# PierfrancescoArdino/C2M

Hardware: AMD Instinct MI355X
Metric: generator train-step frames/sec at 128x256x7 (higher is better)
Workload: dtype f32; 1 GPU; BASELINE configs[1]: 128x256, 7-frame clips (2 in + 5 predicted), batch 8/GPU, fp32, generator fwd+bwd only (no D), VGG loss on, random-init weights; global_batch=8, parallelism=single

## Files before the change

c2m_amd/csrc/conv_common.h:

```cpp
#pragma once
#include "common.h"
#include "dtype.h"
#include "conv_store.h"
#include "conv_types.h"

struct ConvP {
    const float* A;
    const float* X;
    float* Y;
    const float* bias;
    const int4* ktab;
    int M, nk, lda;
    int Npix, To, Ho, Wo;
    int Ti, Hi, Wi;
    int st, sh, sw;
    int in_sc;
    long in_sn, in_st, in_sh;
    long out_sn, out_sc, out_st, out_sh, out_sw, out_off;
    long slab_stride;
    unsigned x_bytes;
    float* Y2;
    int ps_t, ps_y, ps_x, po_t, po_y, po_x, lo_t, lo_y, lo_x, ext_t, ext_y, ext_x;
    long y2_sn, y2_sc, y2_st, y2_sh;
    int iy0, ix0, pty[3], ptx[3], nchunks, cin;
    int ksteps_per_split;
    int reflect, is3d;
    int act;
    float slope;
    int ncls, splits, ktab_cls;
    int xh, yh;
    long a_cls;
    long out_off_c[8];
    int po_c[8][3];
    int g8_nch, g8_ntaps, g8_CB, g8_Mpad;
    unsigned g8_a_bytes, g8_plane_bytes;
    int g8_dbg;
};

struct WgradP {
    const float* dY;
    const float* X;
    float* slab;
    const int4* jtab;
    int M, J;
    int Npix, To, Ho, Wo, Ti, Hi, Wi, st, sh, sw;
    int in_sc;
    long in_sn, in_st, in_sh;
    long dy_sn, dy_sc;
    int pix_per_split;
    int reflect, is3d;
    unsigned x_bytes, dy_bytes;
};

__device__ __forceinline__ int spatial_off(const int4 tp, int ots, int oys, int oxs, int Ti, int Hi, int Wi, int in_st,
                                           int in_sh, int reflect, int is3d) {
    int it = is3d ? ots + tp.x : 0, iy = oys + tp.y, ix = oxs + tp.z;
    bool ok = tp.w != 0;
    if (reflect) {
        if (is3d) { it = it < 0 ? -it : it; it = it >= Ti ? 2 * Ti - 2 - it : it; }
        iy = iy < 0 ? -iy : iy; iy = iy >= Hi ? 2 * Hi - 2 - iy : iy;
        ix = ix < 0 ? -ix : ix; ix = ix >= Wi ? 2 * Wi - 2 - ix : ix;
    } else {
        ok = ok && (unsigned)iy < (unsigned)Hi && (unsigned)ix < (unsigned)Wi;
        if (is3d) ok = ok && (unsigned)it < (unsigned)Ti;
    }
    return ok ? it * in_st + iy * in_sh + ix : -1;
}

template <class P>
__device__ __forceinline__ void decompose_pix(int pix, const P& p, int& n, int& ot, int& oy, int& ox) {
    ox = pix % p.Wo; int r = pix / p.Wo;
    oy = r % p.Ho;   r = r / p.Ho;
    ot = r % p.To;   n = r / p.To;
}

int c2m_launch_gather_nc8(const ConvP& p, int variant, int splits, hipStream_t s);
int c2m_launch_patch(const ConvP& p, int splits, hipStream_t s);
int c2m_launch_patch_bf16(const ConvP& p, int splits, hipStream_t s);
int c2m_launch_thin_fwd(const ConvP& p, int ns, hipStream_t s);
int c2m_launch_thin_rows(const ConvP& p, int kw, int ns, int ntg, int Cin, int xdesc, hipStream_t s);
int c2m_launch_thin_wgrad_rows(const WgradP& p, int kw, int NS, int ntg, int Cin, int ngroups, int S, hipStream_t s);
int c2m_launch_thin_wgrad(WgradP p, int NS, int ngroups, int S, hipStream_t s);
```

c2m_amd/csrc/conv_igemm.hip:

```cpp
#include "conv_common.h"

template <int BM, int BN, int WGM, int WGN, int NS, int U, bool BF = false>
__global__ __launch_bounds__(256) void conv_igemm_kernel(const ConvP p) {
    constexpr int BK = 16, CK = BK / NS, BKU = BK * U;
    constexpr int TM = BM / WGM, TN = BN / WGN, MI = TM / 32, NI = TN / 32;
    constexpr int LDA_S = BM + 4, LDB_S = BN;
    constexpr int BROWS = 256 / BN;
    constexpr int BPASS = BK / BROWS;
    constexpr int A_F4 = BM * BK / 4;
    constexpr int APASS = (A_F4 + 255) / 256;
    static_assert(WGM * WGN == 4 && BN >= 64 && CK % BROWS == 0, "tile");
    static_assert(!BF || BROWS <= 2, "bf16 slot packing is written for BN = 128 / 256");
    __shared__ float sA[BF ? 1 : 2][BF ? 1 : BKU][BF ? 1 : LDA_S];
    __shared__ float sB[BF ? 1 : 2][BF ? 1 : BKU][BF ? 1 : LDB_S];
    __shared__ uint4 hA[BF ? 2 * U * 2 * BM : 1];
    __shared__ uint4 hB[BF ? 2 * U * 2 * BN : 1];

    const int tid = threadIdx.x, lane = tid & 63, wave = tid >> 6;
    const int wm = wave / WGN, wn = wave % WGN;
    const C2mBlock blk = c2m_xcd_block((unsigned)(p.Npix + BN - 1) / BN, (unsigned)(p.M + BM - 1) / BM, 1);
    const int m0 = blk.y * BM, n0 = blk.x * BN;
    const int cls = p.ncls > 1 ? (int)blk.z / p.splits : 0;
    const int split = p.ncls > 1 ? (int)blk.z - cls * p.splits : (int)blk.z;
    const float* __restrict__ Acls = p.A + cls * p.a_cls;
    const int4* __restrict__ ktab = p.ktab + cls * p.ktab_cls;
    const int kt_beg = split * p.ksteps_per_split;
    int kt_end = kt_beg + p.ksteps_per_split; kt_end = kt_end < p.nk ? kt_end : p.nk;

    const int bp = tid % BN;
    const int brow0 = __builtin_amdgcn_readfirstlane(tid / BN);
    int pn, pt, py, px;
    {
        int pix = n0 + bp; pix = pix < p.Npix ? pix : p.Npix - 1;
        decompose_pix(pix, p, pn, pt, py, px);
    }
    const int ots = pt * p.st, oys = py * p.sh, oxs = px * p.sw;
    const int in_st = (int)p.in_st, in_sh = (int)p.in_sh;

    const int akq = (tid & 3) * 4;
    const int arow = tid >> 2;

    f32x16 acc[MI][NI];
#pragma unroll
    for (int i = 0; i < MI; ++i)
#pragma unroll
        for (int j = 0; j < NI; ++j)
#pragma unroll
            for (int r = 0; r < 16; ++r) acc[i][j][r] = 0.f;

    float4 ra[U][APASS];
    float rb[BF ? 1 : U][BF ? 1 : BPASS];
    unsigned short rh[BF ? U : 1][BF ? BPASS : 1];
    constexpr int XES = BF ? 2 : 4;

    const float* __restrict__ aptr[APASS];
#pragma unroll
    for (int s = 0; s < APASS; ++s) {
        int row = m0 + arow + s * 64; row = row < p.M ? row : p.M - 1;
        aptr[s] = Acls + (long)row * p.lda + akq;
    }
    int4 t_hdr, t_tap[NS];
    auto fetch_table = [&](int kt) {
        const int4* __restrict__ kd = ktab + (long)kt * (1 + NS);
        t_hdr = kd[0];
#pragma unroll
        for (int q = 0; q < NS; ++q) t_tap[q] = kd[1 + q];
    };

    const __amdgpu_buffer_rsrc_t xrsrc = __builtin_amdgcn_make_buffer_rsrc(const_cast<float*>(p.X), 0, p.x_bytes, 0x00020000);
    const unsigned img_byte = (unsigned)(pn * (int)p.in_sn) * (unsigned)XES;
    auto load_step = [&](int kt, float4 (&fa)[APASS], float (&fb)[BF ? 1 : BPASS], unsigned short (&fh)[BF ? BPASS : 1]) {
        const bool real = kt < kt_end;
#pragma unroll
        for (int s = 0; s < APASS; ++s) {
            if (A_F4 >= 256 || arow + s * 64 < BM)
                fa[s] = real ? *reinterpret_cast<const float4*>(aptr[s] + kt * BK) : make_float4(0.f, 0.f, 0.f, 0.f);
        }
        const int4 hdr = t_hdr;
        unsigned vo[NS];
#pragma unroll
        for (int q = 0; q < NS; ++q) {
            const int so = spatial_off(t_tap[q], ots, oys, oxs, p.Ti, p.Hi, p.Wi, in_st, in_sh, p.reflect, p.is3d);
            vo[q] = (real && so >= 0) ? img_byte + (unsigned)so * (unsigned)XES : C2M_OOB;
        }
#pragma unroll
        for (int s = 0; s < BPASS; ++s) {
            const int slot = (s * BROWS) / CK;
            const int cc = (s * BROWS) % CK + brow0;
            const int soff = (hdr.x + cc * p.in_sc) * XES;
            if constexpr (BF) fh[s] = __builtin_amdgcn_raw_buffer_load_b16(xrsrc, vo[slot], soff, 0);
            else fb[s] = __builtin_bit_cast(float, __builtin_amdgcn_raw_buffer_load_b32(xrsrc, vo[slot], soff, 0));
        }
        fetch_table(kt + 1 < p.nk ? kt + 1 : p.nk - 1);
    };
    auto load_tile = [&](int kt) {
#pragma unroll
        for (int u = 0; u < U; ++u) load_step(kt + u, ra[u], rb[BF ? 0 : u], rh[BF ? u : 0]);
    };
    auto store_tile = [&](int buf) {
#pragma unroll
        for (int u = 0; u < U; ++u) {
            if constexpr (BF) {
                __bf16* __restrict__ a8 = reinterpret_cast<__bf16*>(hA) + (long)((buf * U + u) * 2) * BM * 8;
#pragma unroll
                for (int s = 0; s < APASS; ++s) {
                    const int r = arow + s * 64;
                    if (A_F4 >= 256 || r < BM) {
                        const float4 v = ra[u][s];
                        if constexpr (BROWS == 1) {
                            bf16x4 q = {(__bf16)v.x, (__bf16)v.y, (__bf16)v.z, (__bf16)v.w};
                            *reinterpret_cast<bf16x4*>(a8 + ((akq >> 3) * BM + r) * 8 + (akq & 7)) = q;
                        } else {
                            bf16x2 e = {(__bf16)v.x, (__bf16)v.z}, o = {(__bf16)v.y, (__bf16)v.w};
                            *reinterpret_cast<bf16x2*>(a8 + (0 * BM + r) * 8 + (akq >> 1)) = e;
                            *reinterpret_cast<bf16x2*>(a8 + (1 * BM + r) * 8 + (akq >> 1)) = o;
                        }
                    }
                }
                uint4* __restrict__ b8 = hB + (long)((buf * U + u) * 2) * BN;
#pragma unroll
                for (int hh = 0; hh < BPASS / 8; ++hh) {
                    bf16x8 q;
#pragma unroll
                    for (int e = 0; e < 8; ++e) q[e] = __builtin_bit_cast(__bf16, rh[u][hh * 8 + e]);
                    const int h = BROWS == 1 ? hh : brow0;
                    b8[h * BN + bp] = __builtin_bit_cast(uint4, q);
                }
            } else {
#pragma unroll
                for (int s = 0; s < APASS; ++s) {
                    int r = arow + s * 64;
                    if (A_F4 >= 256 || r < BM) {
                        sA[buf][u * BK + akq + 0][r] = ra[u][s].x; sA[buf][u * BK + akq + 1][r] = ra[u][s].y;
                        sA[buf][u * BK + akq + 2][r] = ra[u][s].z; sA[buf][u * BK + akq + 3][r] = ra[u][s].w;
                    }
                }
#pragma unroll
                for (int s = 0; s < BPASS; ++s) sB[buf][u * BK + brow0 + s * BROWS][bp] = rb[u][s];
            }
        }
    };

    if (kt_beg < kt_end) {
        fetch_table(kt_beg);
        load_tile(kt_beg);
        store_tile(0);
    }
    __syncthreads();
    int cur = 0;
    for (int kt = kt_beg; kt < kt_end; kt += U) {
        const bool more = kt + U < kt_end;
        constexpr bool IL = !BF && U == 1 && BM < 128;
        if (!IL && more) load_tile(kt + U);
        if constexpr (BF) {
#pragma unroll
            for (int u = 0; u < U; ++u) {
                const uint4* __restrict__ a8 = hA + (long)((cur * U + u) * 2 + (lane >> 5)) * BM;
                const uint4* __restrict__ b8 = hB + (long)((cur * U + u) * 2 + (lane >> 5)) * BN;
                bf16x8 a[MI], b[NI];
#pragma unroll
                for (int i = 0; i < MI; ++i) a[i] = __builtin_bit_cast(bf16x8, a8[wm * TM + i * 32 + (lane & 31)]);
#pragma unroll
                for (int j = 0; j < NI; ++j) b[j] = __builtin_bit_cast(bf16x8, b8[wn * TN + j * 32 + (lane & 31)]);
#pragma unroll
                for (int i = 0; i < MI; ++i)
#pragma unroll
                    for (int j = 0; j < NI; ++j)
                        acc[i][j] = __builtin_amdgcn_mfma_f32_32x32x16_bf16(a[i], b[j], acc[i][j], 0, 0, 0);
            }
        } else if constexpr (IL) {
            float a[BK / 2][MI], b[BK / 2][NI];
#pragma unroll
            for (int kk = 0; kk < BK / 2; ++kk) {
                const int krow = kk * 2 + (lane >> 5);
#pragma unroll
                for (int i = 0; i < MI; ++i) a[kk][i] = sA[cur][krow][wm * TM + i * 32 + (lane & 31)];
#pragma unroll
                for (int j = 0; j < NI; ++j) b[kk][j] = sB[cur][krow][wn * TN + j * 32 + (lane & 31)];
            }
            {
                const int ktl = more ? kt + 1 : kt;
#pragma unroll
                for (int s2 = 0; s2 < APASS; ++s2)
                    if (A_F4 >= 256 || arow + s2 * 64 < BM) ra[0][s2] = *reinterpret_cast<const float4*>(aptr[s2] + ktl * BK);
                const int4 hdr = t_hdr;
                unsigned vo[NS];
#pragma unroll
                for (int q = 0; q < NS; ++q) {
                    const int so = spatial_off(t_tap[q], ots, oys, oxs, p.Ti, p.Hi, p.Wi, in_st, in_sh, p.reflect, p.is3d);
                    vo[q] = so >= 0 ? img_byte + (unsigned)so * 4u : C2M_OOB;
                }
#pragma unroll
                for (int s2 = 0; s2 < BPASS; ++s2) {
                    const int slot = (s2 * BROWS) / CK;
                    const int cc = (s2 * BROWS) % CK + brow0;
                    rb[0][s2] = __builtin_bit_cast(float, __builtin_amdgcn_raw_buffer_load_b32(
                        xrsrc, vo[slot], (hdr.x + cc * p.in_sc) * 4, 0));
                }
            }
#pragma unroll
            for (int kk = 0; kk < BK / 2; ++kk)
#pragma unroll
                for (int i = 0; i < MI; ++i)
#pragma unroll
                    for (int j = 0; j < NI; ++j)
                        acc[i][j] = __builtin_amdgcn_mfma_f32_32x32x2f32(a[kk][i], b[kk][j], acc[i][j], 0, 0, 0);
            constexpr int NMF = (BK / 2) * MI * NI, RPM = (MI + NI + MI * NI - 1) / (MI * NI);
            __builtin_amdgcn_sched_group_barrier(0x100, 2 * (MI + NI), 0);
#pragma unroll
            for (int g = 0; g < NMF; ++g) {
                __builtin_amdgcn_sched_group_barrier(0x008, 1, 0);
                __builtin_amdgcn_sched_group_barrier(0x100, RPM, 0);
                __builtin_amdgcn_sched_group_barrier(0x020, 1, 0);
                __builtin_amdgcn_sched_group_barrier(0x002, 3, 0);
                __builtin_amdgcn_sched_group_barrier(0x004, 2, 0);
            }
            __builtin_amdgcn_sched_barrier(0);
            fetch_table(kt + 2 < p.nk ? kt + 2 : p.nk - 1);
        } else
#pragma unroll
        for (int u = 0; u < U; ++u) {
            float a[BK / 2][MI], b[BK / 2][NI];
#pragma unroll
            for (int kk = 0; kk < BK / 2; ++kk) {
                const int krow = u * BK + kk * 2 + (lane >> 5);
#pragma unroll
                for (int i = 0; i < MI; ++i) a[kk][i] = sA[cur][krow][wm * TM + i * 32 + (lane & 31)];
#pragma unroll
                for (int j = 0; j < NI; ++j) b[kk][j] = sB[cur][krow][wn * TN + j * 32 + (lane & 31)];
            }
#ifdef C2M_IGEMM_SERIAL_FRAGS
            __builtin_amdgcn_sched_barrier(0);
#endif
#pragma unroll
            for (int kk = 0; kk < BK / 2; ++kk) {
#pragma unroll
                for (int i = 0; i < MI; ++i)
#pragma unroll
                    for (int j = 0; j < NI; ++j)
                        acc[i][j] = __builtin_amdgcn_mfma_f32_32x32x2f32(a[kk][i], b[kk][j], acc[i][j], 0, 0, 0);
            }
#ifndef C2M_IGEMM_SERIAL_FRAGS
            {
                constexpr int NMF = (BK / 2) * MI * NI, RPM = (MI + NI + MI * NI - 1) / (MI * NI);
                __builtin_amdgcn_sched_group_barrier(0x100, MI + NI, 0);
#pragma unroll
                for (int g = 0; g < NMF; ++g) {
                    __builtin_amdgcn_sched_group_barrier(0x008, 1, 0);
                    __builtin_amdgcn_sched_group_barrier(0x100, RPM, 0);
                }
            }
#endif
            __builtin_amdgcn_sched_barrier(0);
        }
        if (more) store_tile(cur ^ 1);
        __syncthreads();
        cur ^= 1;
    }

    const bool direct = p.splits == 1;
    const bool yh = BF && p.yh && direct;
    const int yes = yh ? 2 : 4;
    float* __restrict__ Yb = yh ? reinterpret_cast<float*>(reinterpret_cast<bf16_t*>(p.Y) + p.out_off_c[cls])
                                : p.Y + (long)split * p.slab_stride + p.out_off_c[cls];
    const int po_t = p.po_c[cls][0], po_y = p.po_c[cls][1], po_x = p.po_c[cls][2];
    {
        const int row0 = __builtin_amdgcn_readfirstlane(m0 + wm * TM);
        if (row0 + MI * 32 <= p.M) {
            unsigned voff[NI], voff2[NI];
            bool ring = false;
#pragma unroll
            for (int j = 0; j < NI; ++j) {
                const int pix = n0 + wn * TN + j * 32 + (lane & 31);
                int n, ot, oy, ox;
                decompose_pix(pix < p.Npix ? pix : 0, p, n, ot, oy, ox);
                const long e = (long)n * p.out_sn + (long)ot * p.out_st + (long)oy * p.out_sh + (long)ox * p.out_sw +
                               4L * (lane >> 5) * p.out_sc;
                voff[j] = pix < p.Npix ? (unsigned)(e * yes) : 0x80000000u;
                voff2[j] = 0x80000000u;
                if (p.Y2) {
                    const int tp = ot * p.ps_t + po_t - p.lo_t, yp = oy * p.ps_y + po_y - p.lo_y,
                              xp = ox * p.ps_x + po_x - p.lo_x;
                    if (pix < p.Npix && (unsigned)tp < (unsigned)p.ext_t && (unsigned)yp < (unsigned)p.ext_y &&
                        (unsigned)xp < (unsigned)p.ext_x) {
                        const long e2 = (long)n * p.y2_sn + (long)tp * p.y2_st + (long)yp * p.y2_sh + xp +
                                        4L * (lane >> 5) * p.y2_sc;
                        voff2[j] = (unsigned)(e2 * yes);
                        voff[j] = 0x80000000u;
                    }
                }
                ring = ring || voff[j] != 0x80000000u;
            }
            if (p.Y2) c2m_store_tile_fast<MI, NI>(acc, p.Y2, voff2, row0, p.y2_sc, nullptr, false, 0, 0.f, lane, yh);
            if (!p.Y2 || __any(ring))
                c2m_store_tile_fast<MI, NI>(acc, Yb, voff, row0, p.out_sc, p.bias, direct, p.act, p.slope, lane, yh);
            return;
        }
    }
#pragma unroll
    for (int j = 0; j < NI; ++j) {
        const int pix = n0 + wn * TN + j * 32 + (lane & 31);
        if (pix >= p.Npix) continue;
        int n, ot, oy, ox;
        decompose_pix(pix, p, n, ot, oy, ox);
        float* ybase = Yb;
        long yidx = (long)n * p.out_sn + (long)ot * p.out_st + (long)oy * p.out_sh + (long)ox * p.out_sw;
        long row_stride = p.out_sc;
        if (p.Y2) {
            const int tp = ot * p.ps_t + po_t - p.lo_t, yp = oy * p.ps_y + po_y - p.lo_y,
                      xp = ox * p.ps_x + po_x - p.lo_x;
            if ((unsigned)tp < (unsigned)p.ext_t && (unsigned)yp < (unsigned)p.ext_y && (unsigned)xp < (unsigned)p.ext_x) {
                ybase = p.Y2;
                yidx = (long)n * p.y2_sn + (long)tp * p.y2_st + (long)yp * p.y2_sh + xp;
                row_stride = p.y2_sc;
            }
        }
#pragma unroll
        for (int i = 0; i < MI; ++i) {
#pragma unroll
            for (int r = 0; r < 16; ++r) {
                const int row = m0 + wm * TM + i * 32 + (r & 3) + 8 * (r >> 2) + 4 * (lane >> 5);
                if (row < p.M) {
                    float v = acc[i][j][r];
                    if (direct) {
                        if (p.bias) v += p.bias[row];
                        v = c2m_act(v, p.act, p.slope);
                    }
                    if (yh) reinterpret_cast<bf16_t*>(ybase)[yidx + (long)row * row_stride] = (bf16_t)v;
                    else ybase[yidx + (long)row * row_stride] = v;
                }
            }
        }
    }
}

template <class T>
__global__ void splitk_reduce_kernel(const float* __restrict__ slab, T* __restrict__ out,
                                     const float* __restrict__ bias, long total, int S, long chan_stride, int M, int act,
                                     float slope) {
    for (long i = blockIdx.x * (long)blockDim.x + threadIdx.x; i < total; i += (long)gridDim.x * blockDim.x) {
        float acc = 0.f;
        for (int z = 0; z < S; ++z) acc += slab[(long)z * total + i];
        if (bias) acc += bias[(int)((i / chan_stride) % M)];
        c2m_st(out, i, c2m_act(acc, act, slope));
    }
}

template <typename I, class T = float>
__global__ void splitk_reduce_vec_kernel(const float4* __restrict__ slab, T* __restrict__ out,
                                         const float* __restrict__ bias, long total4_, int S, long chan_stride4_, int M,
                                         int act, float slope) {
    const I total4 = (I)total4_, chan_stride4 = (I)chan_stride4_;
    for (I i = blockIdx.x * (I)blockDim.x + threadIdx.x; i < total4; i += (I)gridDim.x * blockDim.x) {
        float4 acc = make_float4(0.f, 0.f, 0.f, 0.f);
        for (int z = 0; z < S; ++z) {
            const float4 v = slab[(long)z * total4_ + i];
            acc.x += v.x; acc.y += v.y; acc.z += v.z; acc.w += v.w;
        }
        if (bias) {
            const float b = bias[(int)((i / chan_stride4) % (I)M)];
            acc.x += b; acc.y += b; acc.z += b; acc.w += b;
        }
        c2m_st4(out + 4 * (long)i, make_float4(c2m_act(acc.x, act, slope), c2m_act(acc.y, act, slope), c2m_act(acc.z, act, slope),
                                               c2m_act(acc.w, act, slope)));
    }
}

template <int BM, int BN, int WGM, int WGN>
static int launch_igemm(const ConvP& p, int ns, int splits, hipStream_t s, bool bf16) {
    dim3 grid((unsigned)c2m_cdiv(p.Npix, BN) * c2m_cdiv(p.M, BM) * splits * p.ncls);
    constexpr int U = 1;
    if (bf16) {
        constexpr int UB = 2;
        switch (ns) {
            case 1: hipLaunchKernelGGL((conv_igemm_kernel<BM, BN, WGM, WGN, 1, UB, true>), grid, dim3(256), 0, s, p); break;
            case 2: hipLaunchKernelGGL((conv_igemm_kernel<BM, BN, WGM, WGN, 2, UB, true>), grid, dim3(256), 0, s, p); break;
            case 4: hipLaunchKernelGGL((conv_igemm_kernel<BM, BN, WGM, WGN, 4, UB, true>), grid, dim3(256), 0, s, p); break;
            default: return (int)hipErrorInvalidValue;
        }
        return (int)hipGetLastError();
    }
    switch (ns) {
        case 1: hipLaunchKernelGGL((conv_igemm_kernel<BM, BN, WGM, WGN, 1, U>), grid, dim3(256), 0, s, p); break;
        case 2: hipLaunchKernelGGL((conv_igemm_kernel<BM, BN, WGM, WGN, 2, 1>), grid, dim3(256), 0, s, p); break;
        case 4: hipLaunchKernelGGL((conv_igemm_kernel<BM, BN, WGM, WGN, 4, 1>), grid, dim3(256), 0, s, p); break;
        default: return (int)hipErrorInvalidValue;
    }
    return (int)hipGetLastError();
}

static void igemm_tile(int M, int& BM, int& BN) {
    if (M <= 32) { BM = 32; BN = 256; }
    else if (M <= 64) { BM = 64; BN = 128; }
    else { BM = 128; BN = 128; }
}

C2M_API int c2m_conv_igemm_splits(int M, int nk, int Npix) {
    int BM, BN;
    igemm_tile(M, BM, BN);
    const long tiles = (long)c2m_cdiv(M, BM) * c2m_cdiv(Npix, BN);
    constexpr long target = 1280;
    if (tiles >= 768 || nk < 8) return 1;
    long S = (target + tiles - 1) / tiles;
    if (S > nk / 4) S = nk / 4;
    if (S > 128) S = 128;
    if (S < 2) return 1;
    const int per = c2m_cdiv(nk, (int)S);
    return c2m_cdiv(nk, per);
}

C2M_API int c2m_conv_igemm(const float* A, const void* X, void* Y, void* Y_interior, const float* bias,
                           const int* ktab, const int64_t* g, int act, float slope, void* stream) {
    C2M_ENTER();
    ConvP p;
    p.A = A; p.X = (const float*)X; p.Y = (float*)Y; p.bias = bias; p.ktab = reinterpret_cast<const int4*>(ktab);
    p.Y2 = (float*)Y_interior;
    p.ps_t = (int)g[C2M_G_PS_T]; p.ps_y = (int)g[C2M_G_PS_Y]; p.ps_x = (int)g[C2M_G_PS_X]; p.po_t = (int)g[C2M_G_PO_T]; p.po_y = (int)g[C2M_G_PO_Y];
    p.po_x = (int)g[C2M_G_PO_X]; p.lo_t = (int)g[C2M_G_LO_T]; p.lo_y = (int)g[C2M_G_LO_Y]; p.lo_x = (int)g[C2M_G_LO_X]; p.ext_t = (int)g[C2M_G_EXT_T];
    p.ext_y = (int)g[C2M_G_EXT_Y]; p.ext_x = (int)g[C2M_G_EXT_X]; p.y2_sn = g[C2M_G_Y2_SN]; p.y2_sc = g[C2M_G_Y2_SC]; p.y2_st = g[C2M_G_Y2_ST]; p.y2_sh = g[C2M_G_Y2_SH];
    p.M = (int)g[C2M_G_M]; p.nk = (int)g[C2M_G_NK]; p.lda = (int)g[C2M_G_LDA];
    p.Npix = (int)g[C2M_G_NPIX]; p.To = (int)g[C2M_G_TO]; p.Ho = (int)g[C2M_G_HO]; p.Wo = (int)g[C2M_G_WO];
    p.Ti = (int)g[C2M_G_TI]; p.Hi = (int)g[C2M_G_HI]; p.Wi = (int)g[C2M_G_WI];
    p.st = (int)g[C2M_G_ST]; p.sh = (int)g[C2M_G_SH]; p.sw = (int)g[C2M_G_SW];
    p.in_sn = g[C2M_G_IN_SN]; p.in_st = g[C2M_G_IN_ST]; p.in_sh = g[C2M_G_IN_SH];
    p.out_sn = g[C2M_G_OUT_SN]; p.out_sc = g[C2M_G_OUT_SC]; p.out_st = g[C2M_G_OUT_ST]; p.out_sh = g[C2M_G_OUT_SH]; p.out_sw = g[C2M_G_OUT_SW]; p.out_off = g[C2M_G_OUT_OFF];
    p.reflect = (int)g[C2M_G_REFLECT]; p.is3d = (int)g[C2M_G_IS3D];
    const int ns = (int)g[C2M_G_NS];
    p.in_sc = (int)g[C2M_G_IN_SC];
    const int splits = (int)g[C2M_G_SPLITS];
    p.slab_stride = g[C2M_G_SLAB_STRIDE];
    if (g[C2M_G_X_BYTES] <= 0 || g[C2M_G_X_BYTES] >= 0x80000000LL) return (int)hipErrorInvalidValue;
    p.x_bytes = (unsigned)g[C2M_G_X_BYTES];
    p.act = act; p.slope = slope;
    p.xh = (int)g[C2M_G_X_TYPE]; p.yh = (int)g[C2M_G_Y_TYPE];
    if ((p.xh | p.yh) & ~1) return (int)hipErrorInvalidValue;
    if (p.M <= 0 || p.Npix <= 0) return 0;
    if (p.nk <= 0 || (p.lda & 3) || (((uintptr_t)A) & 15) || splits < 1) return (int)hipErrorInvalidValue;
    if (p.Y2 && splits != 1) return (int)hipErrorInvalidValue;
    p.ksteps_per_split = c2m_cdiv(p.nk, splits);
    if (!g[C2M_G_PATCH] && c2m_cdiv(p.nk, p.ksteps_per_split) != splits) return (int)hipErrorInvalidValue;
    p.splits = splits;
    p.ncls = g[C2M_G_NCLS] > 1 ? (int)g[C2M_G_NCLS] : 1;
    if (p.ncls > 8) return (int)hipErrorInvalidValue;
    p.a_cls = g[C2M_G_A_CLS]; p.ktab_cls = (int)g[C2M_G_KTAB_CLS];
    p.out_off_c[0] = p.out_off; p.po_c[0][0] = p.po_t; p.po_c[0][1] = p.po_y; p.po_c[0][2] = p.po_x;
    for (int c = 0; c < p.ncls && p.ncls > 1; ++c) {
        p.out_off_c[c] = g[C2M_G_CLS_OUT_OFF + c];
        for (int d = 0; d < 3; ++d) p.po_c[c][d] = (int)g[C2M_G_CLS_PO + 3 * c + d];
    }
    if (p.ncls > 1 && (g[C2M_G_PATCH] || (p.a_cls & 3))) return (int)hipErrorInvalidValue;
    hipStream_t s = (hipStream_t)stream;
    if (g[C2M_G_G8] == 1) {
        const int C = (int)g[C2M_G_CIN], taps = (int)g[C2M_G_TAPS];
        if (g[C2M_G_PRECISION] != 1 || !p.xh || g[C2M_G_PATCH] || C <= 0 || taps <= 0 || taps > 64 || (((uintptr_t)A | (uintptr_t)X) & 15))
            return (int)hipErrorInvalidValue;
        p.g8_nch = c2m_cdiv(C, 16); p.g8_ntaps = taps; p.g8_CB = c2m_cdiv(C, 8); p.g8_Mpad = c2m_cdiv(p.M, 128) * 128;
        if (p.nk != taps * p.g8_nch || p.in_st != (long)p.Hi * p.Wi || p.in_sh != p.Wi) return (int)hipErrorInvalidValue;
        const long plane = (long)p.Ti * p.Hi * p.Wi * 16, ab = (long)p.nk * 2 * p.g8_Mpad * 16;
        if (plane * p.g8_CB > (long)p.x_bytes || p.x_bytes % (plane * p.g8_CB) || ab * p.ncls >= 0x80000000LL)
            return (int)hipErrorInvalidValue;
        p.g8_plane_bytes = (unsigned)plane; p.g8_a_bytes = (unsigned)ab;
        p.g8_dbg = (int)(g[C2M_G_G8_VARIANT] >> 8);
        return c2m_launch_gather_nc8(p, (int)g[C2M_G_G8_VARIANT] & 255, splits, s);
    }
    if (g[C2M_G_PATCH]) {
        if (ns != 1 || p.st != 1 || p.sh != 1 || p.sw != 1) return (int)hipErrorInvalidValue;
        p.iy0 = (int)g[C2M_G_PATCH_IY0]; p.ix0 = (int)g[C2M_G_PATCH_IX0];
        for (int i = 0; i < 3; ++i) { p.pty[i] = (int)g[C2M_G_PATCH_TY + i]; p.ptx[i] = (int)g[C2M_G_PATCH_TX + i]; }
        p.nchunks = p.nk / 9;
        p.cin = (int)g[C2M_G_CIN];
        if (p.nchunks * 9 != p.nk || p.cin <= 0 || p.cin > p.nchunks * 16) return (int)hipErrorInvalidValue;
        p.ksteps_per_split = c2m_cdiv(p.nchunks, splits);
        if (c2m_cdiv(p.nchunks, p.ksteps_per_split) != splits) return (int)hipErrorInvalidValue;
        if (g[C2M_G_PRECISION] == 1) {
            if (p.lda % 128 != 0 || p.lda < p.M || !p.xh) return (int)hipErrorInvalidValue;
            return c2m_launch_patch_bf16(p, splits, s);
        }
        if (p.xh || p.yh) return (int)hipErrorInvalidValue;
        return c2m_launch_patch(p, splits, s);
    }
    if (p.M <= 4 && splits == 1 && p.Npix >= 16384 && !p.Y2 && p.ncls == 1) {
        if (p.xh || p.yh) return (int)hipErrorInvalidValue;
        const int kw = (int)(g[C2M_G_SQUARE_KW] < 0 ? -g[C2M_G_SQUARE_KW] : g[C2M_G_SQUARE_KW]);
        if (p.M <= 3 && (kw == 3 || kw == 7) && !p.is3d && p.To == 1 && p.st == 1 && p.sh == 1 && p.sw == 1 && p.Wo % 4 == 0 &&
            g[C2M_G_TAPS] == kw * kw && g[C2M_G_CIN] > 0 && g[C2M_G_CIN] * kw * kw * 16 <= 48 * 1024) {
            return c2m_launch_thin_rows(p, kw, ns, (int)g[C2M_G_NTG], (int)g[C2M_G_CIN], g[C2M_G_SQUARE_KW] < 0, s);
        }
        return c2m_launch_thin_fwd(p, ns, s);
    }
    const bool bf16 = g[C2M_G_PRECISION] == 1;
    if (bf16 ? !p.xh : (p.xh || p.yh)) return (int)hipErrorInvalidValue;
    if (p.M <= 32)      return launch_igemm<32, 256, 1, 4>(p, ns, splits, s, bf16);
    else if (p.M <= 64) return launch_igemm<64, 128, 2, 2>(p, ns, splits, s, bf16);
    else                return launch_igemm<128, 128, 2, 2>(p, ns, splits, s, bf16);
}

C2M_API int c2m_splitk_reduce(const float* slab, void* out, const float* bias, long total, int splits,
                              long chan_stride, int M, int act, float slope, int dt, void* stream) {
    C2M_ENTER();
    if (total <= 0) return 0;
    const uintptr_t omask = dt == C2M_BF16 ? 7 : 15;
    const bool vec = (total & 3) == 0 && (!bias || (chan_stride & 3) == 0) && (((uintptr_t)slab) & 15) == 0 &&
                     (((uintptr_t)out) & omask) == 0;
    const dim3 grid(c2m_grid(vec ? total / 4 : total, 256));
    hipStream_t s = (hipStream_t)stream;
    C2M_DISPATCH_DT(dt,
        if (vec) {
            if (total / 4 < (1L << 31))
                hipLaunchKernelGGL((splitk_reduce_vec_kernel<unsigned, T>), grid, dim3(256), 0, s, reinterpret_cast<const float4*>(slab),
                                   (T*)out, bias, total / 4, splits, bias ? chan_stride / 4 : 1, M, act, slope);
            else
                hipLaunchKernelGGL((splitk_reduce_vec_kernel<long, T>), grid, dim3(256), 0, s, reinterpret_cast<const float4*>(slab),
                                   (T*)out, bias, total / 4, splits, bias ? chan_stride / 4 : 1, M, act, slope);
        } else {
            hipLaunchKernelGGL(splitk_reduce_kernel<T>, grid, dim3(256), 0, s, slab, (T*)out, bias, total, splits, chan_stride, M,
                               act, slope);
        });
    return (int)hipGetLastError();
}
```

include/c2m_hip.h:

```cpp
#ifndef C2M_HIP_H
#define C2M_HIP_H
#include <stdint.h>
#ifdef __cplusplus
extern "C" {
#endif

enum { C2M_ACT_NONE = 0, C2M_ACT_RELU = 1, C2M_ACT_LRELU = 2, C2M_ACT_SIGMOID = 3 };

#include "c2m_geom.h"
int c2m_abi_version(void);
int c2m_geom_len(void);
int c2m_wino_geom_len(void);

int c2m_conv_igemm_splits(int M, int nk, int Npix);
int c2m_conv_igemm(const float* A, const void* X, void* Y, void* Y_interior, const float* bias, const int* ktab,
                   const int64_t* geom, int act, float slope, void* stream);
int c2m_splitk_reduce(const float* slab, void* out, const float* bias, long total, int splits, long chan_stride,
                      int M, int act, float slope, int dt , void* stream);

int c2m_conv_wgrad_splits(int M, int J, int Npix);
int c2m_conv_wgrad_rows(int M, int ngroups);
int c2m_conv_wgrad(const void* dY, const void* X, float* slab, float* dW, float* db, const int* jtab,
                   const int64_t* geom, void* stream);

int c2m_pack_weights(const float* w, float* packed, const int64_t* g, void* stream);
int c2m_pack_job_bytes(void);
long c2m_pack_job_fill(void* host_job, int type, const void* w, void* packed, const int64_t* g, unsigned first_block);
int c2m_pack_multi(const void* device_jobs, const void* device_blocktab ,
                   int njobs, long total_blocks, void* stream);
long c2m_pack_weights_bf16_patch_bytes(int M, int C);
int c2m_pack_weights_bf16_patch(const float* w, void* out, const int64_t* g, void* stream);
long c2m_pack_weights_bf16_gather_bytes(const int64_t* g);
int c2m_pack_weights_bf16_gather(const float* w, void* out, const int64_t* g, void* stream);

int c2m_nchw_to_nc8(const void* x, void* y, long N, int C, long HW, void* stream);
int c2m_conv_patch_nc8(const void* A, const void* X_nc8, void* Y, void* Y_interior, const float* bias, const int64_t* geom,
                       int act, float slope, void* stream);
long c2m_pack_weights_bf16_s2_bytes(int M, int C);
int c2m_conv_s2_nc8(const void* A, const void* X_nc8, void* Y, const float* bias, int M, int C, long N, int Hi, int Wi, int reflect,
                    int yh, int act, float slope, void* stream);
int c2m_conv_s2_dgrad_nc8(const void* A, const void* dY_nc8, void* T, int M, int K, long N, int Ho, int Wo, int reflect, int th,
                          void* stream);
int c2m_conv3d_nc8(const void* A, const void* X_nc8, void* Y, const float* bias, int M, int C, long N, int T, int H, int W, int reflect,
                   int yh, int act, float slope, void* stream);
int c2m_conv3d_dgrad_nc8(const void* A, const void* dY_nc8, void* target, const int* ptab, int M, int Ctot, int K, long N, int T, int H,
                         int W, int reflect, int th, void* stream);
int c2m_conv_wgrad3d_nc8(const void* dY_nc8, const void* X_nc8, float* slab, float* dW, float* db, int M, int C, long N, int T, int H,
                         int W, int reflect, void* stream);
int c2m_conv_wgrad_nc8_splits(int M, int C, long N, int H, int W, int s2);
long c2m_conv_wgrad_nc8_slab_floats(int M, int C, long N, int H, int W, int s2);
int c2m_conv_wgrad_nc8(const void* dY_nc8, const void* X_nc8, float* slab, float* dW, float* db, int M, int C, long N, int H,
                       int W, int reflect, int s2, void* stream);

long c2m_wino_upack_floats(int M, int K);
int c2m_wino_filter_transform(const float* w, float* upack, int Cout, int Cin, int dgrad, void* stream);
int c2m_wino_regions(int Ho, int Wo);
int c2m_conv_wino(const float* upack, const float* X, float* Y, float* Y_interior, const float* bias,
                  const int64_t* geom, int act, float slope, void* stream);

long c2m_wino4_upack_floats(int M, int K);
int c2m_wino4_filter_transform(const float* w, float* upack, int Cout, int Cin, int dgrad, void* stream);
int c2m_wino4_regions(int Ho, int Wo);
int c2m_conv_wino4(const float* upack, const float* X, float* Y, float* Y_interior, const float* bias,
                   const int64_t* geom, int act, float slope, void* stream);

int c2m_wino_wgrad_splits(int M, int K, int nimg, int H, int W);
int c2m_conv_wino_wgrad(const float* dY, const float* X, float* slab, float* dbslab, float* dW, float* db, int M, int K,
                        int nimg, int H, int W, int reflect, void* stream);
int c2m_conv_wino_wgrad3d(const float* dY, const float* X, float* slab, float* dbslab, float* dW, float* db,
                          int M, int Cin, int N, int T, int H, int W, int reflect, void* stream);

long c2m_ring_pack_floats(int C, int M);
int c2m_ring_pack(const float* w, float* apack, int C, int M, void* stream);
int c2m_reflect_ring_dgrad(const float* apack, const float* w, const float* dY, float* dX, int N, int C, int M, int H, int W,
                           void* stream);
int c2m_reflect_ring_buffer(const float* apack, const float* dY, float* R, int N, int C, int M, int H, int W, int r_l,
                            void* stream);

int c2m_reflect_border_add(const void* dXpad, void* dX, long NC, int T, int H, int W, int pt, int ph, int pw,
                           int dt, void* stream);
int c2m_reflect_fold(const void* dXpad, void* dX, long NC, int T, int H, int W, int pt, int ph, int pw,
                     int dt, void* stream);

long c2m_norm_workspace_floats(int N, int C, long S);
int c2m_norm_stats(const void* x, float* mean, float* invstd, float* running_mean, float* running_var,
                   float* workspace, int N, int C, long S, int mode, float eps, float momentum, int dt, void* stream);
int c2m_norm_set_fused(int on);
int c2m_norm_fwd(const void* x, float* mean, float* invstd, float* running_mean, float* running_var, float* workspace,
                 const float* gamma, const float* beta, const void* gb, void* y, int N, int C, long S, int mode, float eps,
                 float momentum, int act, float slope, int dt, void* stream);
int c2m_norm_stats_rep(const void* x, float* mean, float* invstd, float* running_mean, float* running_var,
                       float* workspace, int N, int C, long S, int mode, float eps, float momentum, int rep, int dt, void* stream);
int c2m_norm_fwd_rep(const void* x, float* mean, float* invstd, float* running_mean, float* running_var, float* workspace,
                     const float* gamma, const float* beta, const void* gb, void* y, int N, int C, long S, int mode, float eps,
                     float momentum, int rep, int act, float slope, int dt, void* stream);
int c2m_norm_apply(const void* x, const float* mean, const float* invstd, const float* gamma, const float* beta,
                   const void* gb, void* y, void* y_nc8, int N, int C, long S, int mode, int act, float slope, int dt, void* stream);
int c2m_norm_bwd(const void* x, const void* gy, const float* mean, const float* invstd, const float* gamma,
                 const float* beta, const void* gb, void* ggb, float* dgamma, float* dbeta, void* dx, void* dx_nc8,
                 float* workspace, int N, int C, long S, int mode, int act, float slope, int dt, void* stream);
int c2m_act_bwd(const void* y, const void* gy, void* gx, long total, int act, float slope, int dt, void* stream);
int c2m_grad_to_nc8(int mode, const void* y, const void* t, const void* gy, const float* gl, void* g_nc8, long N, int C, long S,
                    long count, int act, float slope, void* stream);

int c2m_flow_warp_fwd(const void* img, const float* flow, const float* occ, void* out, int N, int C, int H, int W,
                      int dt, void* stream);
long c2m_flow_warp_bwd_workspace_bytes(int N, int C, int H, int W, int want_gimg, int want_gflow);
int c2m_flow_warp_bwd(const void* img, const float* flow, const float* occ, const void* gout, void* gimg,
                      float* gflow, int N, int C, int H, int W, void* workspace, int dt, void* stream);
int c2m_resize_bilinear(const void* in, void* out, long NC, int Hi, int Wi, int Ho, int Wo, int align,
                        double scale_factor, int dt, void* stream);
int c2m_resize_bilinear_bwd(const void* gout, void* gin, long NC, int Hi, int Wi, int Ho, int Wo, int align, int dt,
                            void* stream);
int c2m_upsample2x_fwd(const void* in, void* out, long NC, int Hi, int Wi, int dt, void* stream);
int c2m_upsample2x_nc8(const void* in_nc8, void* out_nc8, long NCB, int Hi, int Wi, void* stream);
int c2m_upsample2x_bwd(const void* gout, void* gin, long NC, int Hi, int Wi, int dt, void* stream);
int c2m_roi_align_fwd(const float* feat, const float* boxes, float* out, int K, int C, int H, int W, int PH, int PW,
                      float spatial_scale, void* stream);
int c2m_roi_align_bwd(const float* boxes, const float* gout, float* gfeat, int N, int K, int C, int H, int W, int PH,
                      int PW, float spatial_scale, void* stream);
int c2m_maxpool2x2_fwd(const void* in, void* out, long NC, int Hi, int Wi, int dt, void* stream);
int c2m_maxpool2x2_bwd(const void* in, const void* gout, void* gin, long NC, int Hi, int Wi, int dt, void* stream);
int c2m_maxpool2x2_relu_bwd(const void* in, const void* gout, void* gin, long NC, int Hi, int Wi, int dt, void* stream);

int c2m_resample2d_fwd(const float* img, const float* flow, float* out, int N, int C, int H, int W, void* stream);
int c2m_channelnorm_fwd(const float* x, float* out, int N, int C, int H, int W, void* stream);
int c2m_correlation_out_size(int H, int pad, int kernel_size, int max_displacement, int stride1);
int c2m_correlation_fwd(const float* in1, const float* in2, float* out, int N, int C, int H, int W, int pad,
                        int kernel_size, int max_displacement, int stride1, int stride2, void* stream);
int c2m_bias_act(float* x, const float* bias, long N, int C, long HW, int act, float slope, void* stream);

int c2m_sparse_raster(const float* instance, const int* obj_id, const int* obj_batch, const float* thetas, float* bw,
                      float* fw, float* bin, int B, int K, int T, int H, int W, void* stream);
long c2m_occlusion_splat_workspace_bytes(long nimg, int H, int W);
int c2m_occlusion_splat(const float* flow, long sb, long sc, long st, int B, int T, int H, int W, float* occ,
                        float* clip, void* workspace, void* stream);

int c2m_label_warp(const float* flow, long sb, long sc, long st, const float* occ, float threshold, int fill_id,
                   const float* planes_f, int Cf, const int32_t* planes_i, int Ci, int B, int T, int H, int W, float* out_f,
                   int32_t* out_i, void* stream);

long c2m_nearest_fill_workspace_bytes(int B, int T, int H, int W);
int c2m_nearest_fill(const uint8_t* hole, const uint8_t* seed, float* planes_f, long fsb, long fsc, long fst, int Cf,
                     int32_t* planes_i, long isb, long isc, long ist, int Ci, int B, int T, int H, int W, int32_t* unfilled,
                     void* workspace, long workspace_bytes, void* stream);

int c2m_detail_warp(const uint8_t* frame, const float* generated, const float* warped, const float* flow, const float* occ,
                    const int32_t* ids, float threshold, int fill_id, int B, int T, int h, int w, int H, int W, uint8_t* out,
                    int32_t* out_ids, void* stream);

long c2m_frame_quality_workspace_bytes(int B, int T, int H, int W);
int c2m_frame_quality(const void* pred, const void* target, const uint8_t* regions, int form, int B, int C, int T, int H, int W,
                      const long* pred_strides, const long* target_strides, const double* weights, double L, void* workspace,
                      long workspace_bytes, double* out, void* stream);

int c2m_l1_mean_fwd(const void* a, const void* b, const float* mask, float* out, long total, int C, long inner,
                    void* workspace , int dt , void* stream);
int c2m_l1_mean_bwd(const void* a, const void* b, const float* mask, const float* gscale, void* ga, void* gb,
                    long total, int C, long inner, int dt , void* stream);
int c2m_relu_tap_bwd(const void* y, const void* t, const void* gy, const float* gl, void* out, long total,
                     int dt , void* stream);
int c2m_ssim_fwd(const float* x, const float* y, float* out, long NC, int H, int W, void* workspace ,
                 void* stream);
int c2m_ssim_bwd(const float* x, const float* y, const float* gscale, float* gx, float* coef, long NC, int H, int W,
                 void* stream);

int c2m_gat_dense_fwd(const float* xl, const float* xr, const float* att, const float* A, float* out, float* alpha, int N, int H,
                      int C, float negative_slope, void* stream);
long c2m_gat_dense_bwd_workspace_floats(int N, int H, int C);
int c2m_gat_dense_bwd(const float* xl, const float* xr, const float* att, const float* alpha, const float* gout, float* dxl,
                      float* dxr, float* datt, float* workspace, int N, int H, int C, float negative_slope, void* stream);

int c2m_prep_video(const uint8_t* frames_bthwc, float* video_bcthw, int B, int T, int H, int W, void* stream);
int c2m_prep_seg_onehot(const uint8_t* labels_bthw, float* bg_mask, float* fg_mask, int B, int T, int H, int W,
                        void* stream);
int c2m_prep_flow_occ(const uint8_t* occ_bthw, const float* flow_bthwc, float* occ_out, float* flow_out, int B, int T,
                      int H, int W, void* stream);

int c2m_resize_u8(const uint8_t* src, uint8_t* dst, int N, int Hin, int Win, int Hout, int Wout, int C,
                  const int32_t* bounds_x_host, const int32_t* bounds_x, const int32_t* coef_x, int ksx,
                  const int32_t* bounds_y_host, const int32_t* bounds_y, const int32_t* coef_y, int ksy, void* stream);
int c2m_resize_nearest(const void* src, void* dst, int elem_bytes, long N, int Hin, int Win, int Hout, int Wout,
                       const int32_t* index_x_host, const int32_t* index_x, const int32_t* index_y_host, const int32_t* index_y,
                       void* stream);
int c2m_resize_flow(const float* src, float* dst, long N, int Hin, int Win, int Hout, int Wout, const int32_t* bounds_x_host,
                    const int32_t* bounds_x, const float* weight_x, int ksx, const int32_t* bounds_y_host,
                    const int32_t* bounds_y, const float* weight_y, int ksy, void* stream);

int c2m_detect_input(const float* frame, float* out, int B, int C, int H, int W, long stride_b, long stride_c, long stride_h,
                     long stride_w, int scale, int S, void* stream);
int c2m_yolo_candidates(const void* const* heads, const int* grid, const int* nanchors, const float* stride, const float* anchors,
                        int max_anchors, int nheads, int N, int C, float conf_thres, int cap, int* block_count, float* cand,
                        float* score, int* count, void* stream);
int c2m_nms_merge(const float* sorted, const int* count, int N, int cap, float nms_thres, float* dets, int* kept, void* stream);
int c2m_match_detections(const float* dets, const int* kept, int cap, int B, const long* index, int M, const float* roi, int T,
                         const float* x, int tin, int F, const long* batch, long nodes, int scale, int h, int w,
                         double skip_area, double min_area, int* flags, int* boxes, double* err, void* stream);

int c2m_instance_stats(const int32_t* instance, int32_t* table, int B, int T, int t_in, int H, int W, int id_lo, int id_hi,
                       void* stream);
int c2m_instance_compact(const int32_t* table, int32_t* ids, int32_t* boxes, int32_t* count, int32_t* overflow, int B,
                         int t_in, int nid, int id_lo, int min_pixels, int max_nodes, void* stream);

int c2m_instance_link_max_nodes(void);
int c2m_instance_slots(const int32_t* table, int32_t* slot_ids, int32_t* boxes, int32_t* areas, int32_t* count,
                       int32_t* overflow, int planes, int nid, int id_lo, int min_pixels, int max_nodes, void* stream);
int c2m_instance_overlap(const int32_t* ref, const int32_t* frame, const float* flow, const int32_t* ref_slots,
                         const int32_t* ref_count, const int32_t* frame_slots, const int32_t* frame_count, int32_t* pairs,
                         int P, int H, int W, int max_nodes, void* stream);
int c2m_instance_match(const int32_t* pairs, const int32_t* ref_slots, const int32_t* ref_count, const int32_t* frame_slots,
                       const int32_t* frame_count, int32_t* link, int P, int max_nodes, int iou_num, int iou_den,
                       int same_class, void* stream);

int c2m_panoptic_max_top_k(void);
long c2m_panoptic_workspace_bytes(int N, int H, int W, int top_k, int n_things);
int c2m_panoptic_maps(const float* logits, const uint8_t* labels, int C, const float* center, const float* offset,
                      const uint8_t* class_table, const int32_t* thing_classes, int n_things, uint8_t* semantic,
                      int32_t* instance, int32_t* panoptic, int32_t* centers, int32_t* center_count, void* workspace,
                      long workspace_bytes, int N, int H, int W, float threshold, int nms_kernel, int top_k, int label_divisor,
                      int stuff_area, int ignore_label, void* stream);

long c2m_map_quality_workspace_bytes(int N, int num_classes, int label_divisor, int max_pairs);
int c2m_map_quality(const void* pred, const void* gt, int is_u8, const uint8_t* thing_table, int32_t* tp, int32_t* fp,
                    int32_t* fn, double* iou, int64_t* confusion, uint8_t* overflow, void* workspace, long workspace_bytes,
                    int N, int H, int W, int num_classes, int label_divisor, int ignore_label, int max_pairs, void* stream);

int c2m_render_frames(const void* x, int dt, int B, int C, int T, int H, int W, int rows, int cols, int normalize,
                      uint8_t* out, void* stream);
long c2m_render_flow_workspace_bytes(int T);
int c2m_render_flow(const void* flow, int dt, int B, int T, int H, int W, int rows, int cols, int mode, float scale,
                    uint8_t* out, void* workspace, void* stream);
int c2m_render_instances(const int32_t* ids, int B, int T, int H, int W, int rows, int cols, const uint8_t* base,
                         const uint8_t* palette, int P, int id_lo, int id_hi, int alpha, uint8_t* out, void* stream);
int c2m_draw_overlays_max_boxes(void);
int c2m_draw_overlays(uint8_t* sheet, int B, int T, int H, int W, int rows, int cols, const int32_t* boxes,
                      const uint8_t* presence, const uint8_t* box_rgb, int N, const int32_t* points, const int32_t* sample,
                      const int32_t* count, const uint8_t* line_rgb, int D, int P, void* stream);

int c2m_event_create(void** event_out);
int c2m_event_record(void* event, void* stream);
int c2m_event_elapsed_ms(void* start, void* stop, float* ms);
int c2m_event_destroy(void* event);

int c2m_adam_chunk(void);
int c2m_adam_step(const int64_t* table, const int64_t* sizes, const int32_t* blockmap, int ntensors, int nblocks,
                  double beta1, double beta2, double eps, double step_size, double bias_correction2_sqrt, void* stream);

#ifdef __cplusplus
}
#endif
#endif
```

Baseline: 974.8 frames/s.

## Emulate fp32 implicit-GEMM conv with split-bf16 MFMA products

Adds a precision mode to the implicit-GEMM conv kernel that splits each fp32 operand into three bf16 pieces and accumulates six cross products with bf16 MFMA into high and low accumulators. By default (auto) it is used for layers with M>64, or M>32 with nk>=16, replacing the fp32 path. The aim is higher matrix-core throughput than the fp32 path while keeping near-fp32 accuracy. The cost is more LDS space and traffic, extra split arithmetic and register pressure. An env override and launch counters are also added.

```diff
diff --git a/c2m_amd/csrc/conv_common.h b/c2m_amd/csrc/conv_common.h
--- a/c2m_amd/csrc/conv_common.h
+++ b/c2m_amd/csrc/conv_common.h
@@ -67,6 +67,19 @@
     return ok ? it * in_st + iy * in_sh + ix : -1;
 }
 
+__device__ __forceinline__ void c2m_split3(float v, unsigned& p0, unsigned& p1, unsigned& p2) {
+    p0 = __builtin_bit_cast(unsigned, v) & 0xFFFF0000u;
+    const float r = v - __builtin_bit_cast(float, p0);
+    p1 = __builtin_bit_cast(unsigned, r) & 0xFFFF0000u;
+    p2 = __builtin_bit_cast(unsigned, r - __builtin_bit_cast(float, p1));
+}
+__device__ __forceinline__ unsigned c2m_pack_hi(unsigned lo, unsigned hi) { return __builtin_amdgcn_perm(hi, lo, 0x07060302u); }
+
+#define C2M_SPLIT_NPROD 6
+#define C2M_SPLIT_NHIGH 2
+__device__ constexpr int C2M_SPLIT_PA[C2M_SPLIT_NPROD] = {0, 0, 1, 0, 1, 2};
+__device__ constexpr int C2M_SPLIT_PB[C2M_SPLIT_NPROD] = {0, 1, 0, 2, 1, 0};
+
 template <class P>
 __device__ __forceinline__ void decompose_pix(int pix, const P& p, int& n, int& ot, int& oy, int& ox) {
     ox = pix % p.Wo; int r = pix / p.Wo;
diff --git a/c2m_amd/csrc/conv_igemm.hip b/c2m_amd/csrc/conv_igemm.hip
--- a/c2m_amd/csrc/conv_igemm.hip
+++ b/c2m_amd/csrc/conv_igemm.hip
@@ -1,7 +1,11 @@
 #include "conv_common.h"
-
-template <int BM, int BN, int WGM, int WGN, int NS, int U, bool BF = false>
-__global__ __launch_bounds__(256) void conv_igemm_kernel(const ConvP p) {
+#include <stdlib.h>
+#include <string.h>
+
+template <int BM, int BN, int WGM, int WGN, int NS, int U, int PREC = 0>
+__global__ __launch_bounds__(256, (PREC == 2 && BM == 128) ? 2 : 1) void conv_igemm_kernel(const ConvP p) {
+    constexpr bool BF = PREC == 1, SP = PREC == 2, HALF = BF || SP;
+    constexpr int NP = SP ? 3 : 1;
     constexpr int BK = 16, CK = BK / NS, BKU = BK * U;
     constexpr int TM = BM / WGM, TN = BN / WGN, MI = TM / 32, NI = TN / 32;
     constexpr int LDA_S = BM + 4, LDB_S = BN;
@@ -10,11 +14,11 @@
     constexpr int A_F4 = BM * BK / 4;
     constexpr int APASS = (A_F4 + 255) / 256;
     static_assert(WGM * WGN == 4 && BN >= 64 && CK % BROWS == 0, "tile");
-    static_assert(!BF || BROWS <= 2, "bf16 slot packing is written for BN = 128 / 256");
-    __shared__ float sA[BF ? 1 : 2][BF ? 1 : BKU][BF ? 1 : LDA_S];
-    __shared__ float sB[BF ? 1 : 2][BF ? 1 : BKU][BF ? 1 : LDB_S];
-    __shared__ uint4 hA[BF ? 2 * U * 2 * BM : 1];
-    __shared__ uint4 hB[BF ? 2 * U * 2 * BN : 1];
+    static_assert(!HALF || BROWS <= 2, "bf16 slot packing is written for BN = 128 / 256");
+    __shared__ float sA[HALF ? 1 : 2][HALF ? 1 : BKU][HALF ? 1 : LDA_S];
+    __shared__ float sB[HALF ? 1 : 2][HALF ? 1 : BKU][HALF ? 1 : LDB_S];
+    __shared__ uint4 hA[HALF ? 2 * U * NP * 2 * BM : 1];
+    __shared__ uint4 hB[HALF ? 2 * U * NP * 2 * BN : 1];
 
     const int tid = threadIdx.x, lane = tid & 63, wave = tid >> 6;
     const int wm = wave / WGN, wn = wave % WGN;
@@ -47,6 +51,15 @@
         for (int j = 0; j < NI; ++j)
 #pragma unroll
             for (int r = 0; r < 16; ++r) acc[i][j][r] = 0.f;
+    f32x16 lo[SP ? MI : 1][SP ? NI : 1];
+    if constexpr (SP) {
+#pragma unroll
+        for (int i = 0; i < MI; ++i)
+#pragma unroll
+            for (int j = 0; j < NI; ++j)
+#pragma unroll
+                for (int r = 0; r < 16; ++r) lo[i][j][r] = 0.f;
+    }
 
     float4 ra[U][APASS];
     float rb[BF ? 1 : U][BF ? 1 : BPASS];
@@ -126,6 +139,41 @@
                     const int h = BROWS == 1 ? hh : brow0;
                     b8[h * BN + bp] = __builtin_bit_cast(uint4, q);
                 }
+            } else if constexpr (SP) {
+                uint4* __restrict__ a8 = hA + (long)((buf * U + u) * NP * 2) * BM;
+#pragma unroll
+                for (int s = 0; s < APASS; ++s) {
+                    const int r = arow + s * 64;
+                    if (A_F4 >= 256 || r < BM) {
+                        const float4 v = ra[u][s];
+                        unsigned x[3], y[3], z[3], w[3];
+                        c2m_split3(v.x, x[0], x[1], x[2]); c2m_split3(v.y, y[0], y[1], y[2]);
+                        c2m_split3(v.z, z[0], z[1], z[2]); c2m_split3(v.w, w[0], w[1], w[2]);
+#pragma unroll
+                        for (int q = 0; q < 3; ++q) {
+                            unsigned* __restrict__ aq = reinterpret_cast<unsigned*>(a8 + q * 2 * BM);
+                            if constexpr (BROWS == 1) {
+                                *reinterpret_cast<uint2*>(aq + ((akq >> 3) * BM + r) * 4 + ((akq & 7) >> 1)) =
+                                    make_uint2(c2m_pack_hi(x[q], y[q]), c2m_pack_hi(z[q], w[q]));
+                            } else {
+                                aq[(0 * BM + r) * 4 + (akq >> 2)] = c2m_pack_hi(x[q], z[q]);
+                                aq[(1 * BM + r) * 4 + (akq >> 2)] = c2m_pack_hi(y[q], w[q]);
+                            }
+                        }
+                    }
+                }
+                uint4* __restrict__ b8 = hB + (long)((buf * U + u) * NP * 2) * BN;
+#pragma unroll
+                for (int hh = 0; hh < BPASS / 8; ++hh) {
+                    unsigned pc[8][3];
+#pragma unroll
+                    for (int e = 0; e < 8; ++e) c2m_split3(rb[u][hh * 8 + e], pc[e][0], pc[e][1], pc[e][2]);
+                    const int h = BROWS == 1 ? hh : brow0;
+#pragma unroll
+                    for (int q = 0; q < 3; ++q)
+                        b8[(q * 2 + h) * BN + bp] = make_uint4(c2m_pack_hi(pc[0][q], pc[1][q]), c2m_pack_hi(pc[2][q], pc[3][q]),
+                                                               c2m_pack_hi(pc[4][q], pc[5][q]), c2m_pack_hi(pc[6][q], pc[7][q]));
+                }
             } else {
 #pragma unroll
                 for (int s = 0; s < APASS; ++s) {
@@ -150,7 +198,7 @@
     int cur = 0;
     for (int kt = kt_beg; kt < kt_end; kt += U) {
         const bool more = kt + U < kt_end;
-        constexpr bool IL = !BF && U == 1 && BM < 128;
+        constexpr bool IL = PREC == 0 && U == 1 && BM < 128;
         if (!IL && more) load_tile(kt + U);
         if constexpr (BF) {
 #pragma unroll
@@ -167,6 +215,29 @@
 #pragma unroll
                     for (int j = 0; j < NI; ++j)
                         acc[i][j] = __builtin_amdgcn_mfma_f32_32x32x16_bf16(a[i], b[j], acc[i][j], 0, 0, 0);
+            }
+        } else if constexpr (SP) {
+#pragma unroll
+            for (int u = 0; u < U; ++u) {
+                const uint4* __restrict__ a8 = hA + (long)((cur * U + u) * NP * 2 + (lane >> 5)) * BM;
+                const uint4* __restrict__ b8 = hB + (long)((cur * U + u) * NP * 2 + (lane >> 5)) * BN;
+                bf16x8 a[3][MI], b[3][NI];
+#pragma unroll
+                for (int q = 0; q < 3; ++q) {
+#pragma unroll
+                    for (int i = 0; i < MI; ++i) a[q][i] = __builtin_bit_cast(bf16x8, a8[q * 2 * BM + wm * TM + i * 32 + (lane & 31)]);
+#pragma unroll
+                    for (int j = 0; j < NI; ++j) b[q][j] = __builtin_bit_cast(bf16x8, b8[q * 2 * BN + wn * TN + j * 32 + (lane & 31)]);
+                }
+#pragma unroll
+                for (int q = 0; q < C2M_SPLIT_NPROD; ++q)
+#pragma unroll
+                    for (int i = 0; i < MI; ++i)
+#pragma unroll
+                        for (int j = 0; j < NI; ++j) {
+                            f32x16& d = q < C2M_SPLIT_NHIGH ? acc[i][j] : lo[i][j];
+                            d = __builtin_amdgcn_mfma_f32_32x32x16_bf16(a[C2M_SPLIT_PA[q]][i], b[C2M_SPLIT_PB[q]][j], d, 0, 0, 0);
+                        }
             }
         } else if constexpr (IL) {
             float a[BK / 2][MI], b[BK / 2][NI];
@@ -258,6 +329,12 @@
         cur ^= 1;
     }
 
+    if constexpr (SP) {
+#pragma unroll
+        for (int i = 0; i < MI; ++i)
+#pragma unroll
+            for (int j = 0; j < NI; ++j) acc[i][j] += lo[i][j];
+    }
     const bool direct = p.splits == 1;
     const bool yh = BF && p.yh && direct;
     const int yes = yh ? 2 : 4;
@@ -366,18 +443,54 @@
     }
 }
 
+static int direct_math() {
+    const char* e = getenv("C2M_DIRECT_MATH");
+    if (!e || !*e || !strcmp(e, "auto")) return 2;
+    if (!strcmp(e, "fp32")) return 0;
+    if (!strcmp(e, "split")) return 1;
+    return -1;
+}
+
+constexpr int C2M_DIRECT_COUNTS = 9;
+static long direct_counts[C2M_DIRECT_COUNTS];
+static void direct_count(int tile, int ns) {
+    __atomic_fetch_add(&direct_counts[tile * 3 + (ns == 1 ? 0 : (ns == 2 ? 1 : 2))], 1L, __ATOMIC_RELAXED);
+}
+C2M_API int c2m_direct_math_counts(int64_t* out, int reset) {
+    for (int i = 0; i < C2M_DIRECT_COUNTS; ++i) {
+        const long v = reset ? __atomic_exchange_n(&direct_counts[i], 0L, __ATOMIC_RELAXED) : __atomic_load_n(&direct_counts[i], __ATOMIC_RELAXED);
+        if (out) out[i] = v;
+    }
+    return C2M_DIRECT_COUNTS;
+}
+
+static bool igemm_split_pays(int mode, int M, int nk) {
+    if (mode != 2) return mode == 1;
+    return M > 64 || (M > 32 && nk >= 16);
+}
+
 template <int BM, int BN, int WGM, int WGN>
-static int launch_igemm(const ConvP& p, int ns, int splits, hipStream_t s, bool bf16) {
+static int launch_igemm(const ConvP& p, int ns, int splits, hipStream_t s, int prec) {
     dim3 grid((unsigned)c2m_cdiv(p.Npix, BN) * c2m_cdiv(p.M, BM) * splits * p.ncls);
     constexpr int U = 1;
-    if (bf16) {
+    if (prec == 1) {
         constexpr int UB = 2;
         switch (ns) {
-            case 1: hipLaunchKernelGGL((conv_igemm_kernel<BM, BN, WGM, WGN, 1, UB, true>), grid, dim3(256), 0, s, p); break;
-            case 2: hipLaunchKernelGGL((conv_igemm_kernel<BM, BN, WGM, WGN, 2, UB, true>), grid, dim3(256), 0, s, p); break;
-            case 4: hipLaunchKernelGGL((conv_igemm_kernel<BM, BN, WGM, WGN, 4, UB, true>), grid, dim3(256), 0, s, p); break;
+            case 1: hipLaunchKernelGGL((conv_igemm_kernel<BM, BN, WGM, WGN, 1, UB, 1>), grid, dim3(256), 0, s, p); break;
+            case 2: hipLaunchKernelGGL((conv_igemm_kernel<BM, BN, WGM, WGN, 2, UB, 1>), grid, dim3(256), 0, s, p); break;
+            case 4: hipLaunchKernelGGL((conv_igemm_kernel<BM, BN, WGM, WGN, 4, UB, 1>), grid, dim3(256), 0, s, p); break;
             default: return (int)hipErrorInvalidValue;
         }
+        return (int)hipGetLastError();
+    }
+    if (prec == 2) {
+        switch (ns) {
+            case 1: hipLaunchKernelGGL((conv_igemm_kernel<BM, BN, WGM, WGN, 1, U, 2>), grid, dim3(256), 0, s, p); break;
+            case 2: hipLaunchKernelGGL((conv_igemm_kernel<BM, BN, WGM, WGN, 2, U, 2>), grid, dim3(256), 0, s, p); break;
+            case 4: hipLaunchKernelGGL((conv_igemm_kernel<BM, BN, WGM, WGN, 4, U, 2>), grid, dim3(256), 0, s, p); break;
+            default: return (int)hipErrorInvalidValue;
+        }
+        direct_count(BM == 32 ? 0 : (BM == 64 ? 1 : 2), ns);
         return (int)hipGetLastError();
     }
     switch (ns) {
@@ -490,9 +603,12 @@
     }
     const bool bf16 = g[C2M_G_PRECISION] == 1;
     if (bf16 ? !p.xh : (p.xh || p.yh)) return (int)hipErrorInvalidValue;
-    if (p.M <= 32)      return launch_igemm<32, 256, 1, 4>(p, ns, splits, s, bf16);
-    else if (p.M <= 64) return launch_igemm<64, 128, 2, 2>(p, ns, splits, s, bf16);
-    else                return launch_igemm<128, 128, 2, 2>(p, ns, splits, s, bf16);
+    const int math = bf16 ? 0 : direct_math();
+    if (math < 0) return (int)hipErrorInvalidValue;
+    const int prec = bf16 ? 1 : (igemm_split_pays(math, p.M, p.nk) ? 2 : 0);
+    if (p.M <= 32)      return launch_igemm<32, 256, 1, 4>(p, ns, splits, s, prec);
+    else if (p.M <= 64) return launch_igemm<64, 128, 2, 2>(p, ns, splits, s, prec);
+    else                return launch_igemm<128, 128, 2, 2>(p, ns, splits, s, prec);
 }
 
 C2M_API int c2m_splitk_reduce(const float* slab, void* out, const float* bias, long total, int splits,
diff --git a/include/c2m_hip.h b/include/c2m_hip.h
--- a/include/c2m_hip.h
+++ b/include/c2m_hip.h
@@ -69,6 +69,8 @@
                         int nimg, int H, int W, int reflect, void* stream);
 int c2m_conv_wino_wgrad3d(const float* dY, const float* X, float* slab, float* dbslab, float* dW, float* db,
                           int M, int Cin, int N, int T, int H, int W, int reflect, void* stream);
+
+int c2m_direct_math_counts(int64_t* out, int reset);
 
 long c2m_ring_pack_floats(int C, int M);
 int c2m_ring_pack(const float* w, float* apack, int C, int M, void* stream);
```

Result: faster. 1001 frames/s (median of 6 runs) (+2.6%).
